# illiumst/marl-factory-grid

Hardware: AMD Instinct MI355X
Metric: env-steps/sec (whole node), 8-agent 'large' level, batch 65536, 1/2/4/8 MI355X (higher is better)
Workload: dtype f64 rewards/battery/dirt, f64 obs

## Files before the change

__graft_entry__.py:

```python
import os
import subprocess
import sys
from pathlib import Path

ROOT = Path(__file__).resolve().parent
PKG = ROOT / 'marl-factory-grid_amd'
for _p in (PKG, ROOT / 'oracle', ROOT / 'tests'):
    if str(_p) not in sys.path:
        sys.path.insert(0, str(_p))

HIPCC = os.environ.get('HIPCC', '/opt/rocm/bin/hipcc')


UNITS = ['mfg_engine', 'mfg_obs_a', 'mfg_obs_b', 'mfg_obs_c', 'mfg_obs_d', 'mfg_obs_e', 'mfg_obs_f', 'mfg_learn', 'mfg_info', 'mfg_ppo', 'mfg_seac', 'mfg_act']
FLAGS = ['--offload-arch=gfx950', '-O3', '-std=c++17', '-ffp-contract=off', '-fPIC']


def build_hip(force=False, out=None, extra=(), units=None):
    import tempfile
    csrc = PKG / 'csrc'
    src = [csrc / f'{u}.hip' for u in UNITS] + [csrc / 'mfg_kernels.h', csrc / 'mfg_device.h', csrc / 'mfg_info_eval.h',
                                                csrc / 'mfg_learn_device.h', ROOT / 'include' / 'mfg.h',
                                                ROOT / 'include' / 'mfg_learn.h', ROOT / 'include' / 'mfg_info.h']
    varied = set(UNITS if units is None else units) if extra else set()
    if varied - set(UNITS):
        raise ValueError(f'unknown units {sorted(varied - set(UNITS))}: the units are {UNITS}')
    out = Path(out) if out else PKG / 'mfg_amd' / '_lib' / 'libmfg_hip.so'
    out.parent.mkdir(parents=True, exist_ok=True)
    cache = ROOT / 'build' / 'obj'
# ... 117 lines not shown
```

include/mfg.h:

```cpp
#ifndef MFG_H_
#define MFG_H_

#include <stdint.h>

#ifdef __cplusplus
extern "C" {
#endif

#define MFG_ABI_VERSION 5

#define MFG_MAX_AGENTS 128
#define MFG_MAX_ACTIONS 32
#define MFG_MAX_LAYERS 64
#define MFG_MAX_COMBINED 144
#define MFG_MAX_RULES 32
#define MFG_MAX_DOORS 128
#define MFG_MAX_GROUP 128
#define MFG_MAX_POSITIONS 64

enum {
  MFG_ACT_NOOP = 0,
  MFG_ACT_MOVE = 1,
  MFG_ACT_CHARGE = 2,
  MFG_ACT_CLEAN = 3,
// ... 185 lines not shown
  float* emb;
} mfg_packed_obs;

typedef struct mfg_engine mfg_engine;

int mfg_abi_version(void);

int mfg_create(const mfg_spec* spec, int device, int64_t n_envs, mfg_engine** out);
typedef struct mfg_variant {
  int32_t shuffle_table_path;
  int32_t full_temper;
  int32_t bfs_hbm;
  int32_t pairs_lds;
  int32_t render_slots;
  int32_t serial;
} mfg_variant;
int mfg_create_variant(const mfg_spec* spec, int device, int64_t n_envs, const mfg_variant* variant,
                       mfg_engine** out);
int mfg_destroy(mfg_engine* e);
const char* mfg_last_error(const mfg_engine* e);

enum { MFG_INIT_CREATE = 1, MFG_INIT_KEEP_MT = 2, MFG_INIT_NO_RESET = 4 };
int mfg_reset(mfg_engine* e, const uint8_t* mask, void* obs, int obs_dtype, int init, uint64_t seed_base,
              void* stream);

enum { MFG_STEP_AUTO_RESET = 1, MFG_STEP_DEFER_REPLAY = 2 };
int mfg_step(mfg_engine* e, int K, const int32_t* actions, uint32_t philox_seed, uint32_t env_base,
             int64_t step_base, double* reward, uint8_t* done, void* obs, int obs_dtype, uint8_t* ev_act,
             uint8_t* ev_watch, int32_t* ev_misc, int flags, void* stream);

// ... 19 lines not shown
```

marl-factory-grid_amd/csrc/mfg_engine.hip:

```cpp
#include "mfg_kernels.h"

static int wpb_for(size_t lds);

struct mfg_engine {
  int device = 0;
  long long B = 0;
  MfgDevSpec h{};
  MfgDevSpec* d_spec = nullptr;
  std::vector<void*> d_bufs;
  uint8_t* d_state = nullptr;
  int maxpts = 0;
  bool prof = false;
  std::vector<hipEvent_t> ev_free;
  int rd_slot = 0;
  int rd_blocks = 1;
  int rpd_blocks = 1;
  int* rp_hist = nullptr;
  int* rp_order = nullptr;
  uint8_t* rp_key = nullptr;
  hipStream_t aux = nullptr;
  hipEvent_t ev_fork = nullptr, ev_join = nullptr;
  int obs_list_blocks = 1;
  int n_cu = 1;
  bool overlap = false;
  bool replay_each = false;
  int obs_nwv = 1;
  bool replay2 = false;
  struct Mark { int k; hipEvent_t a, b; };
  std::vector<Mark> marks;
  std::string err;
};

static hipEvent_t prof_event(mfg_engine* e) {
  if (!e->ev_free.empty()) {
    hipEvent_t ev = e->ev_free.back();
    e->ev_free.pop_back();
    return ev;
  }
  hipEvent_t ev = nullptr;
  if (hipEventCreate(&ev) != hipSuccess) return nullptr;
  return ev;
}
// ... 252 lines not shown
  for (int f = 0; f < s->n_floor; f++)
    if (s->floor_cells[f] < 0 || s->floor_cells[f] >= s->H * s->W) return fail("floor cell out of range");
  for (int w = 0; w < s->n_walls; w++)
    if (!s->wall_cells || s->wall_cells[w] < 0 || s->wall_cells[w] >= s->H * s->W) return fail("wall cell out of range");
  for (int d = 0; d < s->n_doors; d++)
    if (!s->door_cells || s->door_cells[d] < 0 || s->door_cells[d] >= s->H * s->W) return fail("door cell out of range");
  return 0;
}

static int create_impl(const mfg_spec* s, int device, int64_t n_envs, const mfg_variant& v, mfg_engine** out);
extern "C" int mfg_create_variant(const mfg_spec* s, int device, int64_t n_envs, const mfg_variant* v,
                                  mfg_engine** out) {
  if (!s || !out) return fail("null argument");
  if (n_envs < 1) return fail("n_envs must be >= 1");
  if (validate_spec(s)) return -1;
  const mfg_variant none{0, 0, 0, 0, 0, 0};
  DevGuard g(device);
  return create_impl(s, device, n_envs, v ? *v : none, out);
}
extern "C" int mfg_create(const mfg_spec* s, int device, int64_t n_envs, mfg_engine** out) {
  return mfg_create_variant(s, device, n_envs, nullptr, out);
}

static int create_impl(const mfg_spec* s, int device, int64_t n_envs, const mfg_variant& v, mfg_engine** out) {
  auto* e = new mfg_engine();
  e->device = device;
  e->B = n_envs;
  if (hipSetDevice(device) != hipSuccess) { delete e; return fail("hipSetDevice failed"); }
  MfgDevSpec& h = e->h;
  h.s = *s;
  const int HW = s->H * s->W;
// ... 340 lines not shown
      hipEventCreateWithFlags(&e->ev_join, hipEventDisableTiming) != hipSuccess) {
    delete e; return fail("stream/event creation failed");
  }
  if (h.bfs_bytes && !h.bfs_off) {
    void* pool = nullptr;
    if (hipMalloc(&pool, (size_t)h.bfs_bytes * (size_t)n_envs) != hipSuccess) {
      delete e; return fail("BFS scratch allocation failed");
    }
    e->d_bufs.push_back(pool);
    h.bfs_pool = (uint8_t*)pool;
  }
  if (hipMemcpy(e->d_spec, &h, sizeof(MfgDevSpec), hipMemcpyHostToDevice) != hipSuccess) {
    delete e; return fail("spec upload failed");
  }
  e->maxpts = h.maxpts;
  {
    const int wpb = wpb_for(h.lds_full);
    int per_cu = 0, n_cu = 0;
    const hipError_t occ = h.lane_passes == 2 ? hipOccupancyMaxActiveBlocksPerMultiprocessor(&per_cu, k_resetdone<2>, wpb * 64,
                                                                                 (size_t)h.lds_full * wpb)
                                     : hipOccupancyMaxActiveBlocksPerMultiprocessor(&per_cu, k_resetdone<1>, wpb * 64,
                                                                                 (size_t)h.lds_full * wpb);
    if (occ != hipSuccess ||
        hipDeviceGetAttribute(&n_cu, hipDeviceAttributeMultiprocessorCount, device) != hipSuccess) {
      delete e; return fail("occupancy query failed");
    }
    e->rd_blocks = std::max(1, per_cu) * std::max(1, n_cu);
    if (hipOccupancyMaxActiveBlocksPerMultiprocessor(&per_cu, k_replay_done, 64, (size_t)h.lds_replay_per_wave) !=
        hipSuccess) {
      delete e; return fail("occupancy query failed");
// ... 56 lines not shown
  if (e->ev_fork) (void)hipEventDestroy(e->ev_fork);
  if (e->ev_join) (void)hipEventDestroy(e->ev_join);
  if (e->aux) (void)hipStreamDestroy(e->aux);
  delete e;
  return 0;
}

extern "C" int mfg_layout(const mfg_engine* e, int32_t* out) {
  const MfgLayout& L = e->h.L;
  const int32_t v[] = {L.size, L.o_hdr, L.o_rule_ctr, L.o_agent_pos, L.o_agent_arr, L.o_agent_par, L.o_frozen_org,
                       L.o_frozen_gp, L.o_door, L.o_items, L.o_pods, L.o_drops, L.o_dests, L.o_dirt_pos,
                       L.o_dirt_id, L.o_battery, L.o_frozen_bat, L.o_dirt_amt, L.o_pcg, L.o_mt, L.o_perm,
                       e->h.lmax, e->h.obs_agent_stride, e->h.lds_full, e->h.xchg_ordered, L.o_machines,
                       L.o_maints, L.o_mstate, L.o_mpath, L.o_grank, e->h.dirt_cap, e->h.lds_logic, e->h.lds_obs,
                       e->h.lds_replay_per_wave, e->h.bfs_off, e->h.bfs_bytes, e->h.max_pairs, e->h.scratch_bytes,
                       L.o_logic, e->overlap ? 1 : 0};
  const int n = (int)(sizeof(v) / sizeof(v[0]));
  for (int i = 0; i < n; i++) out[i] = v[i];
  return n;
}

extern "C" void* mfg_state_ptr(mfg_engine* e) { return e ? e->d_state : nullptr; }

static int wpb_for(size_t lds) { return (int)std::max<size_t>(1, std::min<size_t>(MFG_WPB, MFG_LDS_MAX / std::max<size_t>(lds, 1))); }
static unsigned env_grid(const mfg_engine* e, int wpb) { return (unsigned)((e->B + wpb - 1) / wpb); }
#define GEOM(lds) dim3(env_grid(e, wpb_for(lds))), dim3(wpb_for(lds) * 64), (size_t)(lds) * wpb_for(lds)
static const int obs_wpb = MFG_WPB, logic_wpb = 1;
#define GEOMW(lds, W) dim3(env_grid(e, std::min(W, wpb_for(lds)))), dim3(std::min(W, wpb_for(lds)) * 64), \
    (size_t)(lds) * std::min(W, wpb_for(lds))

template <int MP, typename OT, int PK>
// ... 9 lines not shown
  } else if (L.mw) {
    L.W = e->obs_nwv;
    L.lds = (size_t)e->h.lds_obs_shared + (size_t)L.W * e->h.lds_obs_wave;
    const long long per_cu = std::max<long long>(1, (long long)(MFG_LDS_MAX / L.lds));
    L.grid = list ? (unsigned)std::min<long long>(e->B, per_cu * e->n_cu) : (unsigned)e->B;
  } else {
    L.W = std::min(obs_wpb, wpb_for(e->h.lds_obs));
    L.grid = list ? (unsigned)std::min<long long>(env_grid(e, L.W), e->obs_list_blocks) : env_grid(e, L.W);
    L.lds = (size_t)e->h.lds_obs * L.W;
  }
  L.B = e->B;
  L.d_spec = e->d_spec;
  L.d_state = e->d_state;
  L.mm = e->h.mmax || e->h.kmax;
  L.dirt = e->h.dirt_cap != 0;
  return launch_obs_inst<MP, OT, PK>(L, obs, pk, st, skip, list);
}

#define DISPATCH_MP(MPVAL, CALL) \
  switch (MPVAL) {               \
    case 0: { constexpr int MP = 0; CALL; } break; \
    case 4: { constexpr int MP = 4; CALL; } break; \
    case 6: { constexpr int MP = 6; CALL; } break; \
    case 8: { constexpr int MP = 8; CALL; } break; \
    case 10: { constexpr int MP = 10; CALL; } break; \
    case 12: { constexpr int MP = 12; CALL; } break; \
    case 14: { constexpr int MP = 14; CALL; } break; \
    case 16: { constexpr int MP = 16; CALL; } break; \
    case 18: { constexpr int MP = 18; CALL; } break; \
    case 24: { constexpr int MP = 24; CALL; } break; \
// ... 275 lines not shown
```

marl-factory-grid_amd/csrc/mfg_kernels.h:

```cpp
#pragma once
#include <hip/hip_runtime.h>
#ifndef MFG_RESET_OVERLAP
#define MFG_RESET_OVERLAP 1
#endif
#include <stdint.h>
#include <stdio.h>
#include <stdlib.h>
#include <string.h>

#include <string>
#include <vector>
#include <algorithm>
#include <type_traits>

#include "mfg_device.h"

typedef unsigned long long u64;

__device__ __forceinline__ int lane_id() { return (int)__lane_id(); }
__device__ __forceinline__ u64 ballot(bool p) { return (u64)__ballot(p); }
__device__ __forceinline__ int popc(u64 m) { return __popcll(m); }
__device__ __forceinline__ u64 lt_mask() { return (1ull << lane_id()) - 1ull; }
__device__ __forceinline__ int mbcnt(u64 m) {
  return (int)__builtin_amdgcn_mbcnt_hi((uint32_t)(m >> 32), __builtin_amdgcn_mbcnt_lo((uint32_t)m, 0u));
// ... 2099 lines not shown
  wave_sync();
}

template <int MAXPTS>
struct RayLane {
  static_assert(MAXPTS <= 64, "rays of at most 64 points");
  typedef typename std::conditional<(MAXPTS > 32), u64, uint32_t>::type PM;
  static constexpr int RSH = MAXPTS > 32 ? 6 : 5;
  static constexpr int NW = (2 * MAXPTS + 3) / 4;
  uint32_t pk[NW];
  int len;
  PM diag;
  __device__ __forceinline__ int dx(int p) const { return (int)(int8_t)((pk[p >> 1] >> ((p & 1) * 16)) & 0xFF); }
  __device__ __forceinline__ int dy(int p) const { return (int)(int8_t)((pk[p >> 1] >> ((p & 1) * 16 + 8)) & 0xFF); }
  static_assert(MAXPTS % 2 == 0 && NW * 4 == 2 * MAXPTS, "a ray's points are whole dwords");
  __device__ __forceinline__ void load(SpecP S, int ray) {
    const bool has = ray < S->nrays;
    const uint32_t* pts = (const uint32_t*)S->ray_pts + (size_t)(has ? ray : 0) * NW;
#pragma unroll
    for (int q = 0; q < NW; q++) pk[q] = pts[q];
    len = has ? S->ray_len[ray] : 0;
    diag = has ? (PM)S->ray_diag[ray] : (PM)0;
  }
};

typedef __attribute__((address_space(3))) int lds_int;
typedef __attribute__((address_space(1))) int glb_int;
struct PairList {
  lds_int* lds;
  glb_int* glob;
  int nl;
  __device__ __forceinline__ void put(int q, int a, int b, int c) const {
// ... 154 lines not shown
#define MFG_OBS_FLAT_PK 1
#endif
#define CT_CLOSED 0x80000000u
__device__ __forceinline__ uint32_t bperm(int src_lane, uint32_t v) {
  return (uint32_t)__builtin_amdgcn_ds_bpermute(src_lane << 2, (int)v);
}
template <bool LR>
__device__ __forceinline__ void tbl_sync() {
  if constexpr (LR) {
    __builtin_amdgcn_fence(__ATOMIC_SEQ_CST, "agent");
    __builtin_amdgcn_wave_barrier();
  } else {
    wave_sync();
  }
}
template <int MAXPTS, typename OT, bool MM, int PK, bool DIRT, bool MW>
__device__ void build_obs(const Env& e, OT* out_env, int* pair_glob, const ObsPacked& pk, int wv, int nwv,
                          int slot = 0) {
  SpecP S = e.S;
  constexpr bool LR = MAXPTS == 0;
  constexpr int RMP = LR ? 2 : MAXPTS;
  typedef obs_u32<LR> tu32;
  const int A = S->A, H = S->s.H, W = S->s.W, oh = S->oh, ow = S->ow, dd = S->dd, fr = S->fr;
  const bool full = S->r == 0;
  const float invw = 1.0f / (float)ow;
  const int lane = e.lane;
  const bool frozen = e.H(H_FROZEN) != 0;
  build_cmap<MM, MW>(e, wv, nwv);
  const PairList pairs{(lds_int*)e.scratch, (glb_int*)pair_glob, S->pairs_lds};
  int npairs = 0;
  if (!MW || wv == 0) {
    npairs = build_id_pairs<MM>(e, pairs);
    for (int q = lane; q < npairs; q += MFG_WAVE) {
      const int cA = pairs.get(q, 0), cB = pairs.get(q, 1);
      pairs.set(q, 0, ((cA / W) << 16) | (cA % W));
      pairs.set(q, 1, ((cB / W) << 16) | (cB % W));
    }
    if (npairs > S->pairs_lds) mem_sync();
    if (MW && lane == 0) e.hdrp[MFG_HDR_N - 1] = npairs;
  }
  if constexpr (MW) {
    __builtin_amdgcn_fence(__ATOMIC_SEQ_CST, "workgroup");
    __syncthreads();
    npairs = uni(e.hdrp[MFG_HDR_N - 1]);
  }
  uint32_t* fv = LR ? (uint32_t*)(S->obs_pool + (size_t)slot * (size_t)S->obs_slot_bytes)
                    : (uint32_t*)(e.scratch + 3 * S->pairs_lds + (MW ? wv * (S->lds_obs_wave >> 2) : 0));
  const int fw = 2 * fr + 1;
  uint8_t* wsup = (uint8_t*)(fv + S->fv_words);
  const int nsup4 = (dd + 3) >> 2;
  tu32* dsup = (tu32*)((uint32_t*)(wsup + ((dd + 15) & ~15)) + MFG_WAVE);
  const int ndsup = S->dirt_cap >> 5;
  tu32* amw = dsup + ndsup;
  const bool wide = LR && S->A > MFG_WAVE;
  tu32* amw2 = amw + 2 * dd;
  tu32* wdirt = amw + (wide ? 4 : 2) * dd;
  tu32* pq = wdirt + (DIRT ? dd : 0);
  constexpr bool FLAT = MFG_OBS_FLAT && (LR || MAXPTS <= MFG_OBS_FLAT_MAXPTS) &&
                        (PK == 0 || (MFG_OBS_FLAT_PK && (LR || MAXPTS > 8)));
  tu32* ctag = pq + 2 * MFG_WAVE;
  constexpr bool has_dirt = DIRT;
  const float invW = 1.0f / (float)W;
  const int agp = lane < A ? e.agpos()[lane] : -1;
  const int org_l = lane < A ? (frozen ? e.forg()[lane] : agp) : -1;
  const int nT = e.H(H_N_DIRT);
  const int npass = (S->nrays + MFG_WAVE - 1) / MFG_WAVE;
  const int pA0 = lane < npairs ? pairs.get(lane, 0) : 0, pB0 = lane < npairs ? pairs.get(lane, 1) : 0;
  const int agx = agp / W, agy = agp % W, orgx = org_l / W, orgy = org_l % W;
  constexpr bool HOIST_RAYS = !LR && MAXPTS <= 8 && PK == 0;
  constexpr bool PREFETCH_RS = !LR && MAXPTS <= 8 && PK != 2;
  RayLane<RMP> ray0;
  if constexpr (HOIST_RAYS) ray0.load(S, lane);
  int pf_ofl = -1;
  uint32_t pf_b = 0, pf_c = 0, pf_d = 0;
  auto rs_fetch = [&](int ag) {
    const int og = (!LR || ag < MFG_WAVE) ? rl(orgx, ag) * W + rl(orgy, ag) : uni(frozen ? e.forg()[ag] : e.agpos()[ag]);
    pf_ofl = S->ray_static ? uni((int)S->cell_f[og]) : -1;
    if (pf_ofl >= 0) {
      const bool has = lane < S->nrays;
      const uint32_t* rs = S->ray_static + ((size_t)pf_ofl * S->nrays + (has ? lane : 0)) * 3;
      pf_b = has ? rs[0] : 0u;
      pf_c = has ? rs[1] : 0u;
      pf_d = has ? rs[2] : 0u;
    }
  };
  if constexpr (PREFETCH_RS) rs_fetch(MW ? wv : 0);
  for (int a = MW ? wv : 0; a < A; a += MW ? nwv : 1) {
    int apos, ax, ay, ox, oy;
    if (!LR || a < MFG_WAVE) {
      apos = rl(agp, a);
      ax = rl(agx, a); ay = rl(agy, a);
      ox = rl(orgx, a); oy = rl(orgy, a);
    } else {
      apos = uni(e.agpos()[a]);
      const int og = frozen ? uni(e.forg()[a]) : apos;
      ax = apos / W; ay = apos - ax * W;
      ox = og / W; oy = og - ox * W;
    }
    const int wx0 = full ? 0 : ax - S->r, wy0 = full ? 0 : ay - S->r;
    const int ofl = PREFETCH_RS ? pf_ofl : (S->ray_static ? uni((int)S->cell_f[ox * W + oy]) : -1);
    for (int i = lane; i < S->fv_words; i += MFG_WAVE) fv[i] = 0xFFFFFFFFu;
    for (int i = lane; i < nsup4; i += MFG_WAVE) ((uint32_t*)wsup)[i] = 0u;
    for (int i = lane; i < ndsup; i += MFG_WAVE) dsup[i] = 0u;
    for (int i = lane; i < (wide ? 4 : 2) * dd; i += MFG_WAVE) amw[i] = 0u;
    if (has_dirt)
      for (int i = lane; i < dd; i += MFG_WAVE) wdirt[i] = 0u;
    tbl_sync<LR>();
    if (lane < A) {
      const int wx = agx - wx0, wy = agy - wy0;
      if ((unsigned)wx < (unsigned)oh && (unsigned)wy < (unsigned)ow)
        atomicOr((uint32_t*)&amw[2 * (wx * ow + wy) + (lane >> 5)], 1u << (lane & 31));
    }
    if (wide && lane + MFG_WAVE < A) {
      const int p2 = e.agpos()[lane + MFG_WAVE];
      const int wx = p2 / W - wx0, wy = p2 % W - wy0;
      if ((unsigned)wx < (unsigned)oh && (unsigned)wy < (unsigned)ow)
// ... 31 lines not shown
          const uint32_t walked = stopped ? 0u : (stopm ? (((stopm & (0u - stopm)) << 1) - 1u) & lenm : lenm);
          const uint32_t vism = walked & ~cutm;
          stopped |= stopm != 0u;
#pragma unroll
          for (int q = 0; q < 32; q++) {
            const int dx = (int)(int16_t)(pt[q] & 0xFFFFu), dy = (int)(int16_t)(pt[q] >> 16);
            const bool vq = ((vism >> q) & 1u) && (s0 + q > 0);
            atomicMin(vq ? &fv[(dx + fr) * fw + dy + fr] : sink, (uint32_t)((ray_id << 8) + s0 + q));
          }
        }
      }
    } else
    for (int pass = 0; pass < npass; pass++) {
      const int ray_id = pass * MFG_WAVE + lane;
      RayLane<RMP> ray;
      if (HOIST_RAYS && pass == 0) ray = ray0;
      else ray.load(S, ray_id);
      typedef typename RayLane<RMP>::PM PM;
      constexpr int NB = 8 * (int)sizeof(PM);
      PM blkm = 0, cutm = 0;
      if (RMP <= 32 && ofl >= 0) {
        uint32_t dyn;
        if (PREFETCH_RS && pass == 0) {
          blkm = pf_b;
          cutm = pf_c;
          dyn = pf_d;
          if (a + (MW ? nwv : 1) < A) rs_fetch(a + (MW ? nwv : 1));
        } else {
          const bool has = ray_id < S->nrays;
          const uint32_t* rs = S->ray_static + ((size_t)ofl * S->nrays + (has ? ray_id : 0)) * 3;
          blkm = has ? rs[0] : 0u;
          cutm = has ? rs[1] : 0u;
          dyn = has ? rs[2] : 0u;
        }
        while (dyn) {
          const int p = __ffs((int)dyn) - 1;
          dyn &= dyn - 1;
          const int8_t* pt = S->ray_pts + ((size_t)ray_id * S->maxpts + p) * 2;
          const int x = ox + pt[0], y = oy + pt[1];
          blkm |= light_block_bf<MM>(e, x, y) ? ((PM)1 << p) : (PM)0;
          if (p > 0 && ((ray.diag >> p) & 1u)) {
            const bool c = light_block_bf<MM>(e, x, oy + pt[-1]) & light_block_bf<MM>(e, ox + pt[-2], y);
            cutm |= c ? ((PM)1 << p) : (PM)0;
          }
        }
      } else {
#pragma unroll
        for (int p = 0; p < RMP; p++) {
          const int x = ox + ray.dx(p), y = oy + ray.dy(p);
          blkm |= light_block_bf<MM>(e, x, y) ? ((PM)1 << p) : (PM)0;
          if (p > 0) {
            const bool c = light_block_bf<MM>(e, x, oy + ray.dy(p - 1)) & light_block_bf<MM>(e, ox + ray.dx(p - 1), y);
            cutm |= c ? ((PM)1 << p) : (PM)0;
          }
        }
      }
      cutm &= ray.diag;
      const PM lenm = ray.len >= NB ? ~(PM)0 : (((PM)1 << ray.len) - (PM)1);
      const PM stopm = (blkm | cutm) & lenm;
      const PM walked = stopm ? (((stopm & ((PM)0 - stopm)) << 1) - (PM)1) & lenm : lenm;
      const PM vism = walked & ~cutm;
      uint32_t* sink = (uint32_t*)(wsup + ((dd + 15) & ~15)) + lane;
#pragma unroll
      for (int p = 1; p < RMP; p++)
        atomicMin(((vism >> p) & 1u) ? &fv[(ray.dx(p) + fr) * fw + ray.dy(p) + fr] : sink,
                  (uint32_t)((ray_id << RayLane<RMP>::RSH) + p));
    }
    if (lane == 0) fv[fr * fw + fr] = 0u;
    tbl_sync<LR>();
    SupT<tu32> sup;
    sup.items = sup.pods = sup.drops = sup.dests = sup.machines = sup.maints = 0;
    SupHi suph{0, 0, 0, 0};
    sup.wx0 = wx0; sup.wy0 = wy0; sup.oh = oh; sup.ow = ow; sup.W = W;
    sup.wsup = wsup;
    sup.dsup = dsup;
    for (int q0 = 0; q0 < npairs; q0 += MFG_WAVE) {
      const int q = q0 + lane;
      const int pA = q0 == 0 ? pA0 : (q < npairs ? pairs.get(q, 0) : 0);
      const int pB = q0 == 0 ? pB0 : (q < npairs ? pairs.get(q, 1) : 0);
      const int xA = (pA >> 16) - ox + fr, yA = (pA & 0xFFFF) - oy + fr;
// ... 215 lines not shown
        }
#ifndef MFG_OBS_PLAIN_PTS
#define MFG_OBS_PLAIN_PTS 12
#endif
        if constexpr (MW && MAXPTS <= MFG_OBS_PLAIN_PTS) {
          if (inwin) *op = out;
        } else {
          if (inwin) __builtin_nontemporal_store(out, op);
        }
      }
    }
    if constexpr (FLAT) {
      tbl_sync<LR>();
      const int ne = nl * dd;
      const float invdd = 1.0f / (float)dd;
      for (int e0 = 0; e0 < ne; e0 += MFG_WAVE) {
        const int el = min(e0 + lane, ne - 1);
        const int l = (int)(((float)el + 0.5f) * invdd), c = el - l * dd;
        const uint32_t ct = ctag[c];
        const u64 am = (u64)amw[2 * c] | ((u64)amw[2 * c + 1] << 32);
        const uint32_t tf = bperm(l, lr_tf);
        const uint64_t ab = (uint64_t)bperm(l, lr_alo) | ((uint64_t)bperm(l, lr_ahi) << 32);
        const uint32_t ut = tf & 0xFFFFu, fl = tf >> 16;
        int cnt = popc(ct & ut) + popc(am & ab);
        if (wide) {
          const uint64_t ab2 = S->lrec_ab2[(size_t)a * S->lmax + l];
          cnt += popc(((u64)amw2[2 * c] | ((u64)amw2[2 * c + 1] << 32)) & ab2);
        }
        OT out = (OT)cnt;
        if (fl) {
          auto tagv = [&](int tag) -> double {
            if (wide && tag >= MFG_TAG_AGENT0 + MFG_WAVE) {
// ... 62 lines not shown
      if (pk.idx)
        for (int i = pcount + lane; i < pk.cap; i += MFG_WAVE) {
          pk.idx[(size_t)a * pk.cap + i] = 0;
          pk.val[(size_t)a * pk.cap + i] = 0.0f;
        }
      if (pk.cnt && lane == 0) pk.cnt[a] = pcount;
      if (PK == 2 && pk.emb) {
#pragma unroll
        for (int q = 0; q < MFG_MAX_EMB / MFG_WAVE; q++) {
          const int j = q * MFG_WAVE + lane;
          if (q * MFG_WAVE < pk.E && j < pk.E) pk.emb[(size_t)a * pk.E + j] = acc[q];
        }
      }
    }
  }
}

#define MFG_EV_MISC MFG_EV_MISC_N

template <bool RNG, bool MAINT, int NW>
__device__ void env_step(const Env& e, const int (&my_act)[NW], StepOut<NW>& o, int* scratch) {
  SpecP S = e.S;
  const int A = S->A;
#pragma unroll
  for (int h = 0; h < NW; h++) {
    o.my_rew[h] = 0.0; o.my_act_ev[h] = 0; o.my_watch_ev[h] = 0; o.my_slot[h] = -1; o.door_coll[h] = 0;
  }
  o.g_rew = 0.0; o.maint_coll = 0;
  o.respawn_items_value = -1; o.dirt_spawn_value = -1; o.dirt_spawn_valid = 0; o.door_autoclose = 0;
  o.done_mask = 0; o.dest_reached = 0; o.crashed = 0; o.done = 0;
// ... 300 lines not shown
    if (uni(((const int*)(rec + S->L.o_hdr))[H_DONE]) == 0) continue;
    Env e;
    env_full(S, smem + (size_t)wid * S->lds_full, e, env);
    rec_copy(e.lds, rec, S->L.size, e.lane);
    wave_sync();
    env_reset<NW>(e, e.scratch);
    e.setH(H_DONE, 0);
    e.setH(H_DIRT_TOUCH, 0);
    wave_sync();
    rec_copy(rec, e.lds, S->L.size, e.lane);
    wave_sync();
  }
}
#endif

template <int MAXPTS, typename OT, bool MM, int PK, bool DIRT, bool MW = false>
__device__ __forceinline__ void obs_env(SpecP S, uint8_t* slice, const uint8_t* state, long long env, OT* obs,
                                        ObsPacked pk, int wv = 0, int nwv = 1, int slot = 0) {
  Env e;
  e.S = S; e.lds = slice; e.stab = nullptr;
  e.cmap = slice + S->L.o_mt;
  e.scratch = (int*)(slice + S->L.o_mt + (MM ? S->map_bytes : S->map_bytes8));
  e.hdrp = (int*)(slice + S->L.o_hdr);
  e.lane = lane_id();
  const uint8_t* rec = state + (size_t)env * S->L.size;
  if constexpr (MW) {
    const int n16 = S->L.o_mt >> 4;
    for (int i = wv * MFG_WAVE + e.lane; i < n16; i += MFG_WAVE * nwv) ((uint4*)e.lds)[i] = ((const uint4*)rec)[i];
  } else {
    rec_copy(e.lds, rec, S->L.o_mt, e.lane);
  }
  mw_sync<MW>();
  int* pg = S->pair_pool ? S->pair_pool + (size_t)env * 3 * (S->max_pairs - S->pairs_lds) : nullptr;
  if constexpr (PK) {
    const size_t ea = (size_t)env * S->A;
    pk.idx = pk.idx ? pk.idx + ea * pk.cap : nullptr;
    pk.val = pk.val ? pk.val + ea * pk.cap : nullptr;
    pk.cnt = pk.cnt ? pk.cnt + ea : nullptr;
    pk.emb = pk.emb ? pk.emb + ea * pk.E : nullptr;
    build_obs<MAXPTS, OT, MM, PK, DIRT, MW>(e, nullptr, pg, pk, wv, nwv, slot);
  } else {
    build_obs<MAXPTS, OT, MM, PK, DIRT, MW>(e, obs + (size_t)env * S->A * S->obs_agent_stride, pg, pk, wv, nwv, slot);
  }
  if ((!MW || wv == 0) && e.lane == 0 && e.hdrp[H_OVERFLOW])
    ((int*)(state + (size_t)env * S->L.size + S->L.o_hdr))[H_OVERFLOW] = 1;
  if constexpr (MW) __syncthreads();
}

template <int MAXPTS, typename OT, bool MM, int PK, bool DIRT>
static __global__ void __launch_bounds__(MFG_WPB * 64) __attribute__((amdgpu_waves_per_eu(MAXPTS <= 8 ? 7 : 1))) k_obs(const MfgDevSpec* S_, const uint8_t* state, long long B,
                                                      OT* obs, ObsPacked pk, const uint8_t* skip) {
  extern __shared__ __attribute__((aligned(16))) uint8_t smem[];
  SpecP S = (SpecP)S_;
  const int wid = uni(threadIdx.x >> 6);
  const long long env = (long long)blockIdx.x * (blockDim.x >> 6) + wid;
  if (env >= B) return;
  if (skip && skip[env]) return;
  obs_env<MAXPTS, OT, MM, PK, DIRT>(S, smem + (size_t)wid * S->lds_obs, state, env, obs, pk);
}
template <int MAXPTS, typename OT, bool MM, int PK, bool DIRT>
static __global__ void __launch_bounds__(8 * 64) k_obs_mw(const MfgDevSpec* S_, const uint8_t* state, long long B,
                                                           OT* obs, ObsPacked pk, const uint8_t* skip) {
  extern __shared__ __attribute__((aligned(16))) uint8_t smem[];
  SpecP S = (SpecP)S_;
  const long long env = blockIdx.x;
  if (env >= B || (skip && skip[env])) return;
  obs_env<MAXPTS, OT, MM, PK, DIRT, true>(S, smem, state, env, obs, pk, uni(threadIdx.x >> 6), blockDim.x >> 6);
}
template <int MAXPTS, typename OT, bool MM, int PK, bool DIRT>
static __global__ void __launch_bounds__(8 * 64) k_obs_mw_list(const MfgDevSpec* S_, const uint8_t* state,
                                                                long long B, OT* obs, ObsPacked pk,
                                                                const int32_t* list) {
  extern __shared__ __attribute__((aligned(16))) uint8_t smem[];
// ... 7 lines not shown
}
template <typename OT, bool MM, int PK, bool DIRT>
static __global__ void __launch_bounds__(MFG_WAVE) k_obs_lr(const MfgDevSpec* S_, const uint8_t* state, long long B,
                                                            OT* obs, ObsPacked pk, const uint8_t* skip,
                                                            const int32_t* list) {
  extern __shared__ __attribute__((aligned(16))) uint8_t smem[];
  SpecP S = (SpecP)S_;
  const long long n = list ? min((long long)uni(list[0]), B) : B;
  const int slot = (int)blockIdx.x + (list ? S->obs_slots : 0);
  for (long long q = blockIdx.x; q < n; q += gridDim.x) {
    const long long env = list ? (long long)uni(list[2 + q]) : q;
    if (env < 0 || env >= B || (!list && skip && skip[env])) continue;
    obs_env<0, OT, MM, PK, DIRT>(S, smem, state, env, obs, pk, 0, 1, slot);
  }
}
template <int MAXPTS, typename OT, bool MM, int PK, bool DIRT>
static __global__ void __launch_bounds__(MFG_WPB * 64) k_obs_list(const MfgDevSpec* S_, const uint8_t* state, long long B,
                                                           OT* obs, ObsPacked pk, const int32_t* list) {
  extern __shared__ __attribute__((aligned(16))) uint8_t smem[];
  SpecP S = (SpecP)S_;
  const int wid = uni(threadIdx.x >> 6);
  const long long n = min((long long)uni(list[0]), B);
  const long long nw = (long long)gridDim.x * (blockDim.x >> 6);
  for (long long q = (long long)blockIdx.x * (blockDim.x >> 6) + wid; q < n; q += nw) {
    const long long env = uni(list[2 + q]);
    if (env >= 0 && env < B) obs_env<MAXPTS, OT, MM, PK, DIRT>(S, smem + (size_t)wid * S->lds_obs, state, env, obs, pk);
  }
}

__device__ __forceinline__ void replay_env(SpecP S, uint8_t* slice, uint8_t* rec) {
  const int debt = ((const int*)(rec + S->L.o_hdr))[H_DEBT];
  if (debt == 0) return;
  Env e;
  e.S = S;
  e.lds = slice - S->L.o_mt + 4 * RP_HDR_N;
  e.lane = lane_id();
  e.scratch = (int*)(slice + S->replay_sink_off);
  e.cmap = nullptr;
  e.stab = (uint32_t*)(slice + S->replay_stab_off);
  e.hdrp = (int*)slice;
  int* hdr = e.hdr();
// ... 249 lines not shown
                             L.d_spec, L.d_state, L.B, obs, pk, list);                                           \
        else                                                                                                     \
          hipLaunchKernelGGL((k_obs_mw<MP, OT, MMV, PK, DV>), dim3(L.grid), dim3(L.W * 64), L.lds, st, L.d_spec, \
                             L.d_state, L.B, obs, pk, skip);                                                     \
      }                                                                                                          \
    }                                                                                                            \
    if constexpr (MP != 0) if (!mw_done) {                                                                       \
      if (list)                                                                                                  \
        hipLaunchKernelGGL((k_obs_list<MP, OT, MMV, PK, DV>), dim3(L.grid), dim3(L.W * 64), L.lds, st, L.d_spec, \
                           L.d_state, L.B, obs, pk, list);                                                       \
      else                                                                                                       \
        hipLaunchKernelGGL((k_obs<MP, OT, MMV, PK, DV>), dim3(L.grid), dim3(L.W * 64), L.lds, st, L.d_spec,     \
                           L.d_state, L.B, obs, pk, skip);                                                       \
    }                                                                                                            \
  }
#define MFG_INSTANTIATE_OBS(MP)                                                                                  \
  template hipError_t launch_obs_inst<MP, float, 2>(const ObsLaunch&, float*, const ObsPacked&, hipStream_t,      \
                                                    const uint8_t*, const int32_t*);                             \
  template hipError_t launch_obs_inst<MP, float, 1>(const ObsLaunch&, float*, const ObsPacked&, hipStream_t,      \
                                                    const uint8_t*, const int32_t*);                             \
  template hipError_t launch_obs_inst<MP, double, 0>(const ObsLaunch&, double*, const ObsPacked&, hipStream_t,    \
                                                     const uint8_t*, const int32_t*);                            \
  template hipError_t launch_obs_inst<MP, float, 0>(const ObsLaunch&, float*, const ObsPacked&, hipStream_t,      \
                                                    const uint8_t*, const int32_t*);
```

marl-factory-grid_amd/mfg_amd/engine.py:

```python
import ctypes as C
import os
from pathlib import Path

import numpy as np

from . import abi

LIB_PATH = Path(os.environ.get('MFG_HIP_LIB') or Path(__file__).resolve().parent / '_lib' / 'libmfg_hip.so')
EV_MISC = abi.EV_MISC_N
HDR_N = 40
KERNELS = ['k_logic', 'k_resetdone', 'k_obs', 'k_replay', 'k_reset', 'k_obs_done', 'k_replay_sel']

LAYOUT_KEYS = ['size', 'o_hdr', 'o_rule_ctr', 'o_agent_pos', 'o_agent_arr', 'o_agent_par', 'o_frozen_org',
               'o_frozen_gp', 'o_door', 'o_items', 'o_pods', 'o_drops', 'o_dests', 'o_dirt_pos', 'o_dirt_id',
               'o_battery', 'o_frozen_bat', 'o_dirt_amt', 'o_pcg', 'o_mt', 'o_perm', 'lmax', 'obs_agent_stride',
               'lds_full', 'xchg_ordered', 'o_machines', 'o_maints', 'o_mstate', 'o_mpath', 'o_grank', 'dirt_cap',
               'lds_logic', 'lds_obs', 'lds_replay', 'bfs_off', 'bfs_bytes', 'max_pairs', 'scratch_bytes', 'o_logic',
               'reset_overlap']
HDR = {k: i for i, k in enumerate([
    'step', 'episode', 'crashed', 'frozen', 'obs_init', 'debt', 'mt_idx', 'n_items', 'n_pods', 'n_drops',
    'n_dirt', 'n_dests', 'item_base', 'pod_base', 'drop_base', 'dest_base', 'bat_base', 'arrival', 'done',
    'overflow', 'cnt_agent', 'cnt_battery', 'cnt_pod', 'cnt_drop', 'cnt_item', 'cnt_dirt', 'cnt_dest',
    'cnt_machine', 'cnt_maint', 'cnt_gp', 'total_steps', 'n_machines', 'machine_base', 'n_maints', 'maint_base',
    'graph_built', 'dirt_touch'])}

_lib = None


def load_lib():
    global _lib
    if _lib is not None:
        return _lib
    if not LIB_PATH.exists():
# ... 59 lines not shown
    import torch
    n = src.numel() * src.element_size()
    assert dst.numel() * dst.element_size() == n and dst.is_contiguous() and src.is_contiguous()
    st = stream if stream is not None else torch.cuda.current_stream(src.device)
    _check(load_lib().mfg_hbm_copy(_ptr(dst), _ptr(src), n, C.c_void_p(st.cuda_stream)), 'mfg_hbm_copy')


def _check(rc, what, h=None):
    if rc != 0:
        raise RuntimeError(f'{what} failed: {load_lib().mfg_last_error(h).decode()}')


class MfgVariant(C.Structure):
    _fields_ = [('shuffle_table_path', C.c_int32), ('full_temper', C.c_int32), ('bfs_hbm', C.c_int32),
                ('pairs_lds', C.c_int32), ('render_slots', C.c_int32),
                ('serial', C.c_int32)]


class Engine:

    def __init__(self, spec, n_envs, device=0, variant=None):
        import torch
        if not torch.cuda.is_available():
            raise RuntimeError('mfg_amd.Engine needs a GPU (HIP); no CPU fallback exists')
        self.torch = torch
        self.L = load_lib()
        self.spec = spec
        self.B = int(n_envs)
        self.device = torch.device('cuda', device)
        torch.cuda.set_device(self.device)
        h = C.c_void_p()
# ... 274 lines not shown
```

Measured before the change: 35.14 million.

## Specialize observation kernel for common window radii with compile-time geometry

Adds a geometry-specialized observation kernel path, chosen when the spec's view radius is 1-3 with standard ray geometry. Window sizes, ray counts and the visibility-buffer word count become compile-time constants, and ray point loads are reused from the hoisted copy. It also aligns output-store loops to 128-byte boundaries and pins occupancy hints. Costs are an extra compilation unit, many more template instantiations, and a variant flag to fall back to the generic path.

```diff
diff --git a/__graft_entry__.py b/__graft_entry__.py
--- a/__graft_entry__.py
+++ b/__graft_entry__.py
@@ -12,7 +12,7 @@
 HIPCC = os.environ.get('HIPCC', '/opt/rocm/bin/hipcc')
 
 
-UNITS = ['mfg_engine', 'mfg_obs_a', 'mfg_obs_b', 'mfg_obs_c', 'mfg_obs_d', 'mfg_obs_e', 'mfg_obs_f', 'mfg_learn', 'mfg_info', 'mfg_ppo', 'mfg_seac', 'mfg_act']
+UNITS = ['mfg_engine', 'mfg_obs_a', 'mfg_obs_b', 'mfg_obs_c', 'mfg_obs_d', 'mfg_obs_e', 'mfg_obs_f', 'mfg_obs_g', 'mfg_learn', 'mfg_info', 'mfg_ppo', 'mfg_seac', 'mfg_act']
 FLAGS = ['--offload-arch=gfx950', '-O3', '-std=c++17', '-ffp-contract=off', '-fPIC']
 
 
diff --git a/include/mfg.h b/include/mfg.h
--- a/include/mfg.h
+++ b/include/mfg.h
@@ -223,6 +223,7 @@
   int32_t pairs_lds;
   int32_t render_slots;
   int32_t serial;
+  int32_t obs_generic;
 } mfg_variant;
 int mfg_create_variant(const mfg_spec* spec, int device, int64_t n_envs, const mfg_variant* variant,
                        mfg_engine** out);
diff --git a/marl-factory-grid_amd/csrc/mfg_engine.hip b/marl-factory-grid_amd/csrc/mfg_engine.hip
--- a/marl-factory-grid_amd/csrc/mfg_engine.hip
+++ b/marl-factory-grid_amd/csrc/mfg_engine.hip
@@ -26,6 +26,7 @@
   bool replay_each = false;
   int obs_nwv = 1;
   bool replay2 = false;
+  int obs_geo_r = 0;
   struct Mark { int k; hipEvent_t a, b; };
   std::vector<Mark> marks;
   std::string err;
@@ -308,7 +309,7 @@
   if (!s || !out) return fail("null argument");
   if (n_envs < 1) return fail("n_envs must be >= 1");
   if (validate_spec(s)) return -1;
-  const mfg_variant none{0, 0, 0, 0, 0, 0};
+  const mfg_variant none{0, 0, 0, 0, 0, 0, 0};
   DevGuard g(device);
   return create_impl(s, device, n_envs, v ? *v : none, out);
 }
@@ -679,6 +680,14 @@
     delete e; return fail("spec upload failed");
   }
   e->maxpts = h.maxpts;
+  e->obs_geo_r = 0;
+  if (!v.obs_generic && h.r >= 1 && h.r <= 3) {
+    const int R = h.r, d = 2 * R + 1, fw = 2 * d + 1;
+    static const int NRAYS[] = {24, 38, 44};
+    if (h.oh == d && h.ow == d && h.dd == d * d && h.fr == d && h.fv_words == align_up(fw * fw, 4) &&
+        h.maxpts == 2 * R + 2 && h.nrays == NRAYS[R - 1] && h.A <= MFG_WAVE)
+      e->obs_geo_r = R;
+  }
   {
     const int wpb = wpb_for(h.lds_full);
     int per_cu = 0, n_cu = 0;
@@ -765,7 +774,7 @@
                        e->h.lmax, e->h.obs_agent_stride, e->h.lds_full, e->h.xchg_ordered, L.o_machines,
                        L.o_maints, L.o_mstate, L.o_mpath, L.o_grank, e->h.dirt_cap, e->h.lds_logic, e->h.lds_obs,
                        e->h.lds_replay_per_wave, e->h.bfs_off, e->h.bfs_bytes, e->h.max_pairs, e->h.scratch_bytes,
-                       L.o_logic, e->overlap ? 1 : 0};
+                       L.o_logic, e->overlap ? 1 : 0, e->obs_geo_r};
   const int n = (int)(sizeof(v) / sizeof(v[0]));
   for (int i = 0; i < n; i++) out[i] = v[i];
   return n;
@@ -805,6 +814,10 @@
   L.d_state = e->d_state;
   L.mm = e->h.mmax || e->h.kmax;
   L.dirt = e->h.dirt_cap != 0;
+  if constexpr (PK == 0 && (MP == 4 || MP == 6 || MP == 8)) {
+    constexpr int R = MP / 2 - 1;
+    if (e->obs_geo_r == R && !L.mw) return launch_obs_geo<R, OT>(L, obs, st, skip, list);
+  }
   return launch_obs_inst<MP, OT, PK>(L, obs, pk, st, skip, list);
 }
 
diff --git a/marl-factory-grid_amd/csrc/mfg_kernels.h b/marl-factory-grid_amd/csrc/mfg_kernels.h
--- a/marl-factory-grid_amd/csrc/mfg_kernels.h
+++ b/marl-factory-grid_amd/csrc/mfg_kernels.h
@@ -2137,8 +2137,9 @@
   __device__ __forceinline__ int dx(int p) const { return (int)(int8_t)((pk[p >> 1] >> ((p & 1) * 16)) & 0xFF); }
   __device__ __forceinline__ int dy(int p) const { return (int)(int8_t)((pk[p >> 1] >> ((p & 1) * 16 + 8)) & 0xFF); }
   static_assert(MAXPTS % 2 == 0 && NW * 4 == 2 * MAXPTS, "a ray's points are whole dwords");
-  __device__ __forceinline__ void load(SpecP S, int ray) {
-    const bool has = ray < S->nrays;
+  __device__ __forceinline__ void load(SpecP S, int ray) { load(S, ray, S->nrays); }
+  __device__ __forceinline__ void load(SpecP S, int ray, int nrays) {
+    const bool has = ray < nrays;
     const uint32_t* pts = (const uint32_t*)S->ray_pts + (size_t)(has ? ray : 0) * NW;
 #pragma unroll
     for (int q = 0; q < NW; q++) pk[q] = pts[q];
@@ -2323,15 +2324,28 @@
     wave_sync();
   }
 }
-template <int MAXPTS, typename OT, bool MM, int PK, bool DIRT, bool MW>
+template <int R>
+struct ObsGeo {
+  static constexpr int oh = 2 * R + 1, dd = oh * oh, fr = oh, fw = 2 * fr + 1, fv_words = (fw * fw + 3) & ~3;
+  static constexpr int maxpts = 2 * R + 2;
+  static constexpr int nrays = R == 1 ? 24 : (R == 2 ? 38 : 44);
+};
+template <int MAXPTS, typename OT, bool MM, int PK, bool DIRT, bool MW, int R = 0>
 __device__ void build_obs(const Env& e, OT* out_env, int* pair_glob, const ObsPacked& pk, int wv, int nwv,
                           int slot = 0) {
   SpecP S = e.S;
   constexpr bool LR = MAXPTS == 0;
+  constexpr bool GEO = R > 0;
+  static_assert(!GEO || (R <= 3 && MAXPTS == ObsGeo<R>::maxpts && PK == 0 && !MW), "folded window geometry");
+  typedef ObsGeo<GEO ? R : 1> G;
   constexpr int RMP = LR ? 2 : MAXPTS;
   typedef obs_u32<LR> tu32;
-  const int A = S->A, H = S->s.H, W = S->s.W, oh = S->oh, ow = S->ow, dd = S->dd, fr = S->fr;
-  const bool full = S->r == 0;
+  const int A = S->A, H = S->s.H, W = S->s.W, oh = GEO ? G::oh : S->oh, ow = GEO ? G::oh : S->ow,
+            dd = GEO ? G::dd : S->dd, fr = GEO ? G::fr : S->fr;
+#define OBS_GEO_OR(CONST, SPEC) (GEO ? (CONST) : (SPEC))
+#define OBS_NRAYS OBS_GEO_OR(G::nrays, S->nrays)
+#define OBS_FV_WORDS OBS_GEO_OR(G::fv_words, S->fv_words)
+  const bool full = !GEO && S->r == 0;
   const float invw = 1.0f / (float)ow;
   const int lane = e.lane;
   const bool frozen = e.H(H_FROZEN) != 0;
@@ -2356,7 +2370,7 @@
   uint32_t* fv = LR ? (uint32_t*)(S->obs_pool + (size_t)slot * (size_t)S->obs_slot_bytes)
                     : (uint32_t*)(e.scratch + 3 * S->pairs_lds + (MW ? wv * (S->lds_obs_wave >> 2) : 0));
   const int fw = 2 * fr + 1;
-  uint8_t* wsup = (uint8_t*)(fv + S->fv_words);
+  uint8_t* wsup = (uint8_t*)(fv + OBS_FV_WORDS);
   const int nsup4 = (dd + 3) >> 2;
   tu32* dsup = (tu32*)((uint32_t*)(wsup + ((dd + 15) & ~15)) + MFG_WAVE);
   const int ndsup = S->dirt_cap >> 5;
@@ -2373,28 +2387,34 @@
   const int agp = lane < A ? e.agpos()[lane] : -1;
   const int org_l = lane < A ? (frozen ? e.forg()[lane] : agp) : -1;
   const int nT = e.H(H_N_DIRT);
-  const int npass = (S->nrays + MFG_WAVE - 1) / MFG_WAVE;
+  const int npass = (OBS_NRAYS + MFG_WAVE - 1) / MFG_WAVE;
   const int pA0 = lane < npairs ? pairs.get(lane, 0) : 0, pB0 = lane < npairs ? pairs.get(lane, 1) : 0;
   const int agx = agp / W, agy = agp % W, orgx = org_l / W, orgy = org_l % W;
   constexpr bool HOIST_RAYS = !LR && MAXPTS <= 8 && PK == 0;
   constexpr bool PREFETCH_RS = !LR && MAXPTS <= 8 && PK != 2;
   RayLane<RMP> ray0;
-  if constexpr (HOIST_RAYS) ray0.load(S, lane);
+  if constexpr (HOIST_RAYS) ray0.load(S, lane, OBS_NRAYS);
   int pf_ofl = -1;
   uint32_t pf_b = 0, pf_c = 0, pf_d = 0;
   auto rs_fetch = [&](int ag) {
     const int og = (!LR || ag < MFG_WAVE) ? rl(orgx, ag) * W + rl(orgy, ag) : uni(frozen ? e.forg()[ag] : e.agpos()[ag]);
     pf_ofl = S->ray_static ? uni((int)S->cell_f[og]) : -1;
     if (pf_ofl >= 0) {
-      const bool has = lane < S->nrays;
-      const uint32_t* rs = S->ray_static + ((size_t)pf_ofl * S->nrays + (has ? lane : 0)) * 3;
+      const bool has = lane < OBS_NRAYS;
+      const uint32_t* rs = S->ray_static + ((size_t)pf_ofl * OBS_NRAYS + (has ? lane : 0)) * 3;
       pf_b = has ? rs[0] : 0u;
       pf_c = has ? rs[1] : 0u;
       pf_d = has ? rs[2] : 0u;
     }
   };
   if constexpr (PREFETCH_RS) rs_fetch(MW ? wv : 0);
+  const int lane_outer = lane;
   for (int a = MW ? wv : 0; a < A; a += MW ? nwv : 1) {
+#ifndef MFG_OBS_GEO_LANE_OPAQUE
+#define MFG_OBS_GEO_LANE_OPAQUE 1
+#endif
+    int lane = lane_outer;
+    if constexpr (GEO && MFG_OBS_GEO_LANE_OPAQUE) asm volatile("" : "+v"(lane));
     int apos, ax, ay, ox, oy;
     if (!LR || a < MFG_WAVE) {
       apos = rl(agp, a);
@@ -2406,9 +2426,9 @@
       ax = apos / W; ay = apos - ax * W;
       ox = og / W; oy = og - ox * W;
     }
-    const int wx0 = full ? 0 : ax - S->r, wy0 = full ? 0 : ay - S->r;
+    const int wx0 = full ? 0 : ax - OBS_GEO_OR(R, S->r), wy0 = full ? 0 : ay - OBS_GEO_OR(R, S->r);
     const int ofl = PREFETCH_RS ? pf_ofl : (S->ray_static ? uni((int)S->cell_f[ox * W + oy]) : -1);
-    for (int i = lane; i < S->fv_words; i += MFG_WAVE) fv[i] = 0xFFFFFFFFu;
+    for (int i = lane; i < OBS_FV_WORDS; i += MFG_WAVE) fv[i] = 0xFFFFFFFFu;
     for (int i = lane; i < nsup4; i += MFG_WAVE) ((uint32_t*)wsup)[i] = 0u;
     for (int i = lane; i < ndsup; i += MFG_WAVE) dsup[i] = 0u;
     for (int i = lane; i < (wide ? 4 : 2) * dd; i += MFG_WAVE) amw[i] = 0u;
@@ -2470,8 +2490,11 @@
     for (int pass = 0; pass < npass; pass++) {
       const int ray_id = pass * MFG_WAVE + lane;
       RayLane<RMP> ray;
-      if (HOIST_RAYS && pass == 0) ray = ray0;
-      else ray.load(S, ray_id);
+      if constexpr (GEO) {
+        ray.len = ray0.len;
+        ray.diag = ray0.diag;
+      } else if (HOIST_RAYS && pass == 0) ray = ray0;
+      else ray.load(S, ray_id, OBS_NRAYS);
       typedef typename RayLane<RMP>::PM PM;
       constexpr int NB = 8 * (int)sizeof(PM);
       PM blkm = 0, cutm = 0;
@@ -2483,8 +2506,8 @@
           dyn = pf_d;
           if (a + (MW ? nwv : 1) < A) rs_fetch(a + (MW ? nwv : 1));
         } else {
-          const bool has = ray_id < S->nrays;
-          const uint32_t* rs = S->ray_static + ((size_t)ofl * S->nrays + (has ? ray_id : 0)) * 3;
+          const bool has = ray_id < OBS_NRAYS;
+          const uint32_t* rs = S->ray_static + ((size_t)ofl * OBS_NRAYS + (has ? ray_id : 0)) * 3;
           blkm = has ? rs[0] : 0u;
           cutm = has ? rs[1] : 0u;
           dyn = has ? rs[2] : 0u;
@@ -2492,7 +2515,7 @@
         while (dyn) {
           const int p = __ffs((int)dyn) - 1;
           dyn &= dyn - 1;
-          const int8_t* pt = S->ray_pts + ((size_t)ray_id * S->maxpts + p) * 2;
+          const int8_t* pt = S->ray_pts + ((size_t)ray_id * OBS_GEO_OR(G::maxpts, S->maxpts) + p) * 2;
           const int x = ox + pt[0], y = oy + pt[1];
           blkm |= light_block_bf<MM>(e, x, y) ? ((PM)1 << p) : (PM)0;
           if (p > 0 && ((ray.diag >> p) & 1u)) {
@@ -2501,6 +2524,7 @@
           }
         }
       } else {
+        if constexpr (GEO) ray.load(S, ray_id, OBS_NRAYS);
 #pragma unroll
         for (int p = 0; p < RMP; p++) {
           const int x = ox + ray.dx(p), y = oy + ray.dy(p);
@@ -2519,7 +2543,7 @@
       uint32_t* sink = (uint32_t*)(wsup + ((dd + 15) & ~15)) + lane;
 #pragma unroll
       for (int p = 1; p < RMP; p++)
-        atomicMin(((vism >> p) & 1u) ? &fv[(ray.dx(p) + fr) * fw + ray.dy(p) + fr] : sink,
+        atomicMin(((vism >> p) & 1u) ? &fv[((GEO ? ray0 : ray).dx(p) + fr) * fw + (GEO ? ray0 : ray).dy(p) + fr] : sink,
                   (uint32_t)((ray_id << RayLane<RMP>::RSH) + p));
     }
     if (lane == 0) fv[fr * fw + fr] = 0u;
@@ -2765,8 +2789,14 @@
       tbl_sync<LR>();
       const int ne = nl * dd;
       const float invdd = 1.0f / (float)dd;
-      for (int e0 = 0; e0 < ne; e0 += MFG_WAVE) {
-        const int el = min(e0 + lane, ne - 1);
+#ifndef MFG_OBS_GEO_ALIGN
+#define MFG_OBS_GEO_ALIGN 128
+#endif
+      int e_first = 0;
+      if constexpr (GEO && MFG_OBS_GEO_ALIGN > 0)
+        e_first = -(int)(((size_t)out_a / sizeof(OT)) & (MFG_OBS_GEO_ALIGN / sizeof(OT) - 1));
+      for (int e0 = e_first; e0 < ne; e0 += MFG_WAVE) {
+        const int el = min((GEO && MFG_OBS_GEO_ALIGN > 0) ? max(e0 + lane, 0) : e0 + lane, ne - 1);
         const int l = (int)(((float)el + 0.5f) * invdd), c = el - l * dd;
         const uint32_t ct = ctag[c];
         const u64 am = (u64)amw[2 * c] | ((u64)amw[2 * c + 1] << 32);
@@ -2859,6 +2889,9 @@
       }
     }
   }
+#undef OBS_NRAYS
+#undef OBS_FV_WORDS
+#undef OBS_GEO_OR
 }
 
 #define MFG_EV_MISC MFG_EV_MISC_N
@@ -3189,7 +3222,7 @@
 }
 #endif
 
-template <int MAXPTS, typename OT, bool MM, int PK, bool DIRT, bool MW = false>
+template <int MAXPTS, typename OT, bool MM, int PK, bool DIRT, bool MW = false, int R = 0>
 __device__ __forceinline__ void obs_env(SpecP S, uint8_t* slice, const uint8_t* state, long long env, OT* obs,
                                         ObsPacked pk, int wv = 0, int nwv = 1, int slot = 0) {
   Env e;
@@ -3213,17 +3246,20 @@
     pk.val = pk.val ? pk.val + ea * pk.cap : nullptr;
     pk.cnt = pk.cnt ? pk.cnt + ea : nullptr;
     pk.emb = pk.emb ? pk.emb + ea * pk.E : nullptr;
-    build_obs<MAXPTS, OT, MM, PK, DIRT, MW>(e, nullptr, pg, pk, wv, nwv, slot);
+    build_obs<MAXPTS, OT, MM, PK, DIRT, MW, R>(e, nullptr, pg, pk, wv, nwv, slot);
   } else {
-    build_obs<MAXPTS, OT, MM, PK, DIRT, MW>(e, obs + (size_t)env * S->A * S->obs_agent_stride, pg, pk, wv, nwv, slot);
+    build_obs<MAXPTS, OT, MM, PK, DIRT, MW, R>(e, obs + (size_t)env * S->A * S->obs_agent_stride, pg, pk, wv, nwv, slot);
   }
   if ((!MW || wv == 0) && e.lane == 0 && e.hdrp[H_OVERFLOW])
     ((int*)(state + (size_t)env * S->L.size + S->L.o_hdr))[H_OVERFLOW] = 1;
   if constexpr (MW) __syncthreads();
 }
 
-template <int MAXPTS, typename OT, bool MM, int PK, bool DIRT>
-static __global__ void __launch_bounds__(MFG_WPB * 64) __attribute__((amdgpu_waves_per_eu(MAXPTS <= 8 ? 7 : 1))) k_obs(const MfgDevSpec* S_, const uint8_t* state, long long B,
+#ifndef MFG_OBS_GEO_WPE
+#define MFG_OBS_GEO_WPE 7
+#endif
+template <int MAXPTS, typename OT, bool MM, int PK, bool DIRT, int R = 0>
+static __global__ void __launch_bounds__(MFG_WPB * 64) __attribute__((amdgpu_waves_per_eu(R > 0 ? MFG_OBS_GEO_WPE : (MAXPTS <= 8 ? 7 : 1)))) k_obs(const MfgDevSpec* S_, const uint8_t* state, long long B,
                                                       OT* obs, ObsPacked pk, const uint8_t* skip) {
   extern __shared__ __attribute__((aligned(16))) uint8_t smem[];
   SpecP S = (SpecP)S_;
@@ -3231,7 +3267,7 @@
   const long long env = (long long)blockIdx.x * (blockDim.x >> 6) + wid;
   if (env >= B) return;
   if (skip && skip[env]) return;
-  obs_env<MAXPTS, OT, MM, PK, DIRT>(S, smem + (size_t)wid * S->lds_obs, state, env, obs, pk);
+  obs_env<MAXPTS, OT, MM, PK, DIRT, false, R>(S, smem + (size_t)wid * S->lds_obs, state, env, obs, pk);
 }
 template <int MAXPTS, typename OT, bool MM, int PK, bool DIRT>
 static __global__ void __launch_bounds__(8 * 64) k_obs_mw(const MfgDevSpec* S_, const uint8_t* state, long long B,
@@ -3269,7 +3305,7 @@
     obs_env<0, OT, MM, PK, DIRT>(S, smem, state, env, obs, pk, 0, 1, slot);
   }
 }
-template <int MAXPTS, typename OT, bool MM, int PK, bool DIRT>
+template <int MAXPTS, typename OT, bool MM, int PK, bool DIRT, int R = 0>
 static __global__ void __launch_bounds__(MFG_WPB * 64) k_obs_list(const MfgDevSpec* S_, const uint8_t* state, long long B,
                                                            OT* obs, ObsPacked pk, const int32_t* list) {
   extern __shared__ __attribute__((aligned(16))) uint8_t smem[];
@@ -3279,7 +3315,8 @@
   const long long nw = (long long)gridDim.x * (blockDim.x >> 6);
   for (long long q = (long long)blockIdx.x * (blockDim.x >> 6) + wid; q < n; q += nw) {
     const long long env = uni(list[2 + q]);
-    if (env >= 0 && env < B) obs_env<MAXPTS, OT, MM, PK, DIRT>(S, smem + (size_t)wid * S->lds_obs, state, env, obs, pk);
+    if (env >= 0 && env < B)
+      obs_env<MAXPTS, OT, MM, PK, DIRT, false, R>(S, smem + (size_t)wid * S->lds_obs, state, env, obs, pk);
   }
 }
 
@@ -3559,6 +3596,30 @@
                            L.d_state, L.B, obs, pk, skip);                                                       \
     }                                                                                                            \
   }
+template <int R, typename OT>
+hipError_t launch_obs_geo(const ObsLaunch& L, OT* obs, hipStream_t st, const uint8_t* skip, const int32_t* list);
+#define MFG_OBS_GEO_LAUNCH_IF(MMV, DV)                                                                           \
+  if (L.mm == MMV && L.dirt == DV) {                                                                             \
+    if (list)                                                                                                    \
+      hipLaunchKernelGGL((k_obs_list<2 * R + 2, OT, MMV, 0, DV, R>), dim3(L.grid), dim3(L.W * 64), L.lds, st,    \
+                         L.d_spec, L.d_state, L.B, obs, ObsPacked{}, list);                                      \
+    else                                                                                                         \
+      hipLaunchKernelGGL((k_obs<2 * R + 2, OT, MMV, 0, DV, R>), dim3(L.grid), dim3(L.W * 64), L.lds, st,         \
+                         L.d_spec, L.d_state, L.B, obs, ObsPacked{}, skip);                                      \
+  }
+#define MFG_DEFINE_LAUNCH_OBS_GEO                                                                                \
+  template <int R, typename OT>                                                                                  \
+  hipError_t launch_obs_geo(const ObsLaunch& L, OT* obs, hipStream_t st, const uint8_t* skip,                    \
+                            const int32_t* list) {                                                               \
+    MFG_OBS_GEO_LAUNCH_IF(true, true) else MFG_OBS_GEO_LAUNCH_IF(true, false)                                    \
+    else MFG_OBS_GEO_LAUNCH_IF(false, true) else MFG_OBS_GEO_LAUNCH_IF(false, false)                             \
+    return hipGetLastError();                                                                                    \
+  }
+#define MFG_INSTANTIATE_OBS_GEO(R)                                                                               \
+  template hipError_t launch_obs_geo<R, double>(const ObsLaunch&, double*, hipStream_t, const uint8_t*,          \
+                                                const int32_t*);                                                 \
+  template hipError_t launch_obs_geo<R, float>(const ObsLaunch&, float*, hipStream_t, const uint8_t*,            \
+                                               const int32_t*);
 #define MFG_INSTANTIATE_OBS(MP)                                                                                  \
   template hipError_t launch_obs_inst<MP, float, 2>(const ObsLaunch&, float*, const ObsPacked&, hipStream_t,      \
                                                     const uint8_t*, const int32_t*);                             \
diff --git a/marl-factory-grid_amd/csrc/mfg_obs_g.hip b/marl-factory-grid_amd/csrc/mfg_obs_g.hip
--- /dev/null
+++ b/marl-factory-grid_amd/csrc/mfg_obs_g.hip
@@ -0,0 +1,7 @@
+#define MFG_OBS_UNIT
+#include "mfg_kernels.h"
+
+MFG_DEFINE_LAUNCH_OBS_GEO
+MFG_INSTANTIATE_OBS_GEO(1)
+MFG_INSTANTIATE_OBS_GEO(2)
+MFG_INSTANTIATE_OBS_GEO(3)
diff --git a/marl-factory-grid_amd/mfg_amd/engine.py b/marl-factory-grid_amd/mfg_amd/engine.py
--- a/marl-factory-grid_amd/mfg_amd/engine.py
+++ b/marl-factory-grid_amd/mfg_amd/engine.py
@@ -16,7 +16,7 @@
                'o_battery', 'o_frozen_bat', 'o_dirt_amt', 'o_pcg', 'o_mt', 'o_perm', 'lmax', 'obs_agent_stride',
                'lds_full', 'xchg_ordered', 'o_machines', 'o_maints', 'o_mstate', 'o_mpath', 'o_grank', 'dirt_cap',
                'lds_logic', 'lds_obs', 'lds_replay', 'bfs_off', 'bfs_bytes', 'max_pairs', 'scratch_bytes', 'o_logic',
-               'reset_overlap']
+               'reset_overlap', 'obs_geo_r']
 HDR = {k: i for i, k in enumerate([
     'step', 'episode', 'crashed', 'frozen', 'obs_init', 'debt', 'mt_idx', 'n_items', 'n_pods', 'n_drops',
     'n_dirt', 'n_dests', 'item_base', 'pod_base', 'drop_base', 'dest_base', 'bat_base', 'arrival', 'done',
@@ -106,7 +106,7 @@
 class MfgVariant(C.Structure):
     _fields_ = [('shuffle_table_path', C.c_int32), ('full_temper', C.c_int32), ('bfs_hbm', C.c_int32),
                 ('pairs_lds', C.c_int32), ('render_slots', C.c_int32),
-                ('serial', C.c_int32)]
+                ('serial', C.c_int32), ('obs_generic', C.c_int32)]
 
 
 class Engine:
```

Result: faster. 36.79 million (median of 6 runs) (+4.7%).
